# kevroy314/respmon

Measured on AMD Instinct MI355X. Metric: Eulerian-calibration frames/sec on 1080p x 256 buffer; achieved HBM GB/s, higher is better.
Workload: dtype f64

## Files before the change

### include/respmon_hip_debug.h

```cpp
#ifndef RESPMON_HIP_DEBUG_H
#define RESPMON_HIP_DEBUG_H

#include "respmon_hip.h"

#ifdef __cplusplus
extern "C" {
#endif

#define RM_FLAG_TINY_STORE 4u
#define RM_FLAG_TINY_STRIPS 8u
#define RM_FLAG_FF_PER_LEVEL 512u

int rm_debug_set(rm_ctx *ctx, const char *key, long long value);

int rm_debug_counters(rm_ctx *ctx, long long *out_host, void *stream);

const char *rm_debug_kernel_source_stamp(void);

int rm_debug_workspace(rm_ctx *ctx, const char *name, void *out_host, size_t bytes, void *stream);

int rm_debug_window_rows(rm_ctx *ctx, const rm_window *win, int row0, int nrows, double *out_host, void *stream);

#define RM_HOST_MARKS 5
int rm_debug_host_timeline(rm_ctx *ctx, double *out_host);

#define RM_ROI_PATH_NONE 0
#define RM_ROI_PATH_ONE_BLOB 1
#define RM_ROI_PATH_SCAN 2
#define RM_ROI_PATH_LABELLED 3
#define RM_ROI_PATH_AREA_BOUND 4
int rm_debug_roi_path(rm_ctx *ctx, int *path_out);

#ifdef __cplusplus
}
#endif
#endif
```

### respmon_amd/_capi.py

```python
import ctypes
import os

RM_OK = 0
RM_NO_CONTOUR = 1
RM_SPARSE_FALLBACK = 2
RM_COMM_ID_BYTES = 128
RM_EXCHANGE_SPARSE, RM_EXCHANGE_DENSE = 1, 2
RM_E_BADARG = -1
RM_E_UNSUPPORTED = -4
RM_E_COMM = -6
RM_E_BUSY = -7
RM_LOCATE_TICKETS = 2
RM_MAX_ROIS = 64
RM_U8, RM_F16, RM_F32, RM_F64 = 0, 1, 2, 3
RM_BGR8 = 4
RM_FLAG_NO_PRUNE = 1
RM_FLAG_UNFUSED_DOWN = 2
RM_FLAG_TINY_STORE = 4
RM_FLAG_TINY_STRIPS = 8
RM_FLAG_UNFUSED_SMALL = 16
RM_FLAG_CONTOUR_CLIP_FRAME = 32
RM_FLAG_FILTER_LAPLACIANS = 64
RM_FLAG_DENSE_SUM = 128
RM_FLAG_SPARSE_SUM = 256
RM_FLAG_FF_PER_LEVEL = 512

_c = ctypes
_vp, _i, _d, _sz, _u = _c.c_void_p, _c.c_int, _c.c_double, _c.c_size_t, _c.c_uint

SIGNATURES = {
    "rm_ctx_create": (_i, [_i, _c.POINTER(_vp)]),
    "rm_ctx_destroy": (_i, [_vp]),
    "rm_last_error_string": (_c.c_char_p, []),
    "rm_abi_version": (_i, []),
    "rm_ctx_workspace_bytes": (_sz, [_vp]),
    "rm_debug_set": (_i, [_vp, _c.c_char_p, _c.c_longlong]),
    "rm_profile_enable": (_i, [_vp, _i]),
    "rm_set_contour_clip_frame": (_i, [_vp, _i]),
    "rm_set_contour_labelling": (_i, [_vp, _i]),
    "rm_get_contour_clip_frame": (_i, [_vp, _c.POINTER(_i)]),
    "rm_get_contour_labelling": (_i, [_vp, _c.POINTER(_i)]),
    "rm_contour_stats": (_i, [_vp, _vp, _vp]),
    "rm_profile_read": (_i, [_vp, _vp, _c.POINTER(_i)]),
    "rm_debug_counters": (_i, [_vp, _vp, _vp]),
    "rm_debug_workspace": (_i, [_vp, _c.c_char_p, _vp, _c.c_size_t, _vp]),
    "rm_debug_kernel_source_stamp": (_c.c_char_p, []),
    "rm_debug_host_timeline": (_i, [_vp, _vp]),
    "rm_debug_roi_path": (_i, [_vp, _vp]),
    "rm_uint8_to_float": (_i, [_vp, _vp, _vp, _sz, _vp]),
    "rm_float_to_uint8": (_i, [_vp, _vp, _vp, _sz, _vp]),
    "rm_pyr_down": (_i, [_vp, _vp, _i, _i, _i, _i, _vp, _vp]),
    "rm_pyr_up": (_i, [_vp, _vp, _i, _i, _i, _vp, _i, _i, _i, _vp, _vp]),
    "rm_create_laplacian_video_pyramid": (_i, [_vp, _vp, _i, _i, _i, _i, _i, _c.POINTER(_vp), _vp]),
    "rm_collapse_laplacian_video_pyramid": (_i, [_vp, _c.POINTER(_vp), _i, _i, _i, _i, _vp, _vp]),
    "rm_temporal_bandpass_filter_fft": (_i, [_vp, _vp, _i, _sz, _d, _d, _d, _d, _vp, _vp]),
    "rm_temporal_operator": (_i, [_i, _d, _d, _d, _vp, _c.POINTER(_i), _c.POINTER(_i)]),
    "rm_time_average": (_i, [_vp, _vp, _i, _i, _sz, _vp, _vp]),
    "rm_lfilter": (_i, [_vp, _vp, _i, _sz, _vp, _vp, _i, _d, _vp, _vp]),
    "rm_threshold_mask": (_i, [_vp, _vp, _sz, _d, _vp, _vp, _vp]),
    "rm_eulerian_magnification_bandpass": (_i, [_vp, _vp, _i, _i, _i, _i, _d, _d, _d, _d, _i, _i, _d, _vp, _vp, _vp, _vp]),
    "rm_magnify": (_i, [_vp, _vp, _i, _i, _i, _i, _d, _d, _d, _d, _i, _i, _vp, _i, _vp]),
    "rm_magnify_bgr": (_i, [_vp, _vp, _i, _i, _i, _d, _d, _d, _d, _i, _i, _vp, _vp]),
    "rm_calibrate": (_i, [_vp, _vp, _i, _i, _i, _i, _d, _d, _d, _d, _i, _i, _d, _u, _vp, _vp, _vp]),
    "rm_heatmap_to_roi": (_i, [_vp, _vp, _i, _i, _i, _vp, _vp, _vp, _vp]),
    "rm_heat_sparse_packet_doubles": (_sz, [_i]),
    "rm_heat_sparse_pack": (_i, [_vp, _vp, _i, _i, _i, _vp, _vp]),
    "rm_heat_sparse_merge_roi": (_i, [_vp, _vp, _i, _i, _i, _i, _i, _i, _vp, _vp, _vp]),
    "rm_heat_sparse_tiles_needed": (_i, [_vp, _vp]),
    "rm_locate": (_i, [_vp, _vp, _i, _i, _i, _i, _d, _d, _d, _d, _i, _i, _d, _i, _u, _vp, _vp]),
    "rm_heatmap_to_rois": (_i, [_vp, _vp, _i, _i, _i, _i, _d, _vp, _vp, _c.POINTER(_i), _vp]),
    "rm_locate_multi": (_i, [_vp, _vp, _i, _i, _i, _i, _d, _d, _d, _d, _i, _i, _d, _i, _u, _i, _d, _vp, _vp, _c.POINTER(_i), _vp]),
    "rm_locate_submit": (_i, [_vp, _vp, _i, _i, _i, _i, _d, _d, _d, _d, _i, _i, _d, _i, _u, _vp, _vp]),
    "rm_locate_result": (_i, [_vp, _i, _vp]),
    "rm_shard_layout": (_i, [_i, _i, _i, _i, _c.POINTER(_sz)]),
    "rm_shard_layout_flags": (_i, [_i, _i, _i, _i, _c.c_uint, _c.POINTER(_sz)]),
    "rm_shard_pyramid": (_i, [_vp, _vp, _i, _i, _i, _i, _i, _i, _u, _vp, _vp]),
    "rm_shard_collapse": (_i, [_vp, _vp, _i, _i, _i, _i, _i, _d, _d, _d, _d, _i, _i, _d, _u, _vp, _vp]),
    "rm_shard_heat": (_i, [_vp, _vp, _d, _vp, _vp]),
    "rm_shard_finish": (_i, [_vp, _vp, _i, _i, _i, _i, _vp, _vp, _vp]),
    "rm_window_create": (_i, [_vp, _i, _i, _i, _i, _i, _u, _c.POINTER(_vp)]),
    "rm_window_destroy": (_i, [_vp]),
# ... 71 lines not shown
```

### respmon_amd/csrc/rm_ctx.hip

```cpp
#include "rm_internal.h"

using namespace rm;

static thread_local std::string g_err;

int fail(int code, const char *fmt, ...)
{
    char buf[512];
    va_list ap;
    va_start(ap, fmt);
    vsnprintf(buf, sizeof buf, fmt, ap);
    va_end(ap);
    g_err = buf;
    return code;
}

int ws_get(rm_ctx *ctx, const std::string &name, size_t bytes, void **out)
{
    DevBuf &b = ctx->bufs[name];
    if (b.cap < bytes) {
        if (b.p) {
            for (LocateTicket &t : ctx->tickets)
                if (t.active && t.done) HIP_TRY(hipEventSynchronize(t.done));
            const char *c = (const char *)ctx->dbg_cS, *p0 = (const char *)b.p;
            if (c && c >= p0 && c < p0 + b.cap) ctx->dbg_cS = nullptr;
            HIP_TRY(hipFree(b.p));
        }
        b.p = nullptr; b.cap = 0;
        size_t cap = (bytes + 255) / 256 * 256;
        HIP_TRY(hipMalloc(&b.p, cap));
        b.cap = cap;
    }
    *out = b.p;
    return RM_OK;
}

int ctx_stream_ok(rm_ctx *ctx, void *stream, const char *who)
{
    for (const LocateTicket &t : ctx->tickets)
        if (t.active && t.stream != (hipStream_t)stream)
            return fail(RM_E_BUSY, "%s: a rm_locate_submit of this context is in flight on another stream (fetch it with rm_locate_result first, or "
                                   "use its stream)", who);
    return RM_OK;
}

extern "C" int rm_debug_roi_path(rm_ctx *ctx, int *path_out)
{
    if (!ctx || !path_out) return fail(RM_E_BADARG, "rm_debug_roi_path: bad argument");
    *path_out = ctx->roi_path;
    return RM_OK;
}

extern "C" int rm_debug_host_timeline(rm_ctx *ctx, double *out)
{
    if (!ctx || !out) return fail(RM_E_BADARG, "rm_debug_host_timeline: bad argument");
    for (int i = 0; i < RM_HOST_MARKS; ++i) out[i] = ctx->host_marks[i];
    return RM_OK;
}

extern "C" int rm_abi_version(void) { return 1; }
extern "C" const char *rm_last_error_string(void) { return g_err.c_str(); }

extern "C" int rm_ctx_create(int device, rm_ctx **out)
{
    if (!out) return fail(RM_E_BADARG, "rm_ctx_create: out is NULL");
    HIP_TRY(hipSetDevice(device));
    rm_ctx *c = new rm_ctx();
    c->device = device;
    HIP_TRY(hipMalloc((void **)&c->d_state, sizeof(CollapseState)));
    HIP_TRY(hipHostMalloc((void **)&c->h_state, sizeof(CollapseState), hipHostMallocDefault));
    *out = c;
    return RM_OK;
}

extern "C" int rm_ctx_destroy(rm_ctx *ctx)
{
    if (!ctx) return RM_OK;
    (void)hipSetDevice(ctx->device);
    for (LocateTicket &t : ctx->tickets) {
        if (t.active && t.done) (void)hipEventSynchronize(t.done);
        if (t.done) (void)hipEventDestroy(t.done);
    }
// ... 21 lines not shown
    DebugKnobs &d = ctx->dbg;
    const std::string k(key);
    if (k == "temporal_valu") d.temporal_valu = (int)value;
    else if (k == "temporal_wide") d.temporal_wide = (int)value;
    else if (k == "dc_lds_front_end") d.dc_lds_front_end = (int)value;
    else if (k == "bgr_unfused") d.bgr_unfused = (int)value;
    else if (k == "no_fused_bounds") d.no_fused_bounds = (int)value;
    else if (k == "bounds_table_bytes") d.bounds_table_bytes = value;
    else if (k == "bounds_scalar") d.bounds_scalar = (int)value;
    else if (k == "bounds_l1") d.bounds_l1 = (int)value;
    else if (k == "bounds_up1") d.bounds_up1 = (int)value;
    else if (k == "dense_wf_list") d.dense_wf_list = (int)value;
    else if (k == "bounds_l1_rows") d.bounds_l1_rows = (int)value;
    else if (k == "dense_rows") d.dense_rows = (int)value;
    else if (k == "dense_general") d.dense_general = (int)value;
    else if (k == "dense_wave") d.dense_wave = (int)value;
    else if (k == "dense_frames") d.dense_frames = (int)value;
    else if (k == "dense_split") d.dense_split = (int)value;
    else if (k == "dc_segs") d.dc_segs = (int)value;
    else if (k == "dc_wpg") d.dc_wpg = (int)value;
    else if (k == "dc_split") d.dc_split = (int)value;
    else if (k == "dc_prio") d.dc_prio = (int)value;
    else if (k == "dc_prio_shift") d.dc_prio_shift = (int)value;
    else if (k == "store_slots") d.store_slots = value;
    else if (k == "store_default_slots") d.store_default_slots = value;
    else if (k == "collapse_fused") d.collapse_fused = (int)value;
    else if (k == "eval_fast") d.eval_fast = (int)value;
    else if (k == "exchange_dense") d.exchange_dense = (int)value;
    else if (k == "host_simple_shape") d.host_simple_shape = (int)value;
    else if (k == "host_area_bound") d.host_area_bound = (int)value;
    else if (k == "label_lazy") d.label_lazy = (int)value;
    else if (k == "heat_rows") d.heat_rows = (int)value;
    else if (k == "ff_parts") d.ff_parts = (int)value;
    else if (k == "heat_const_tiles") d.heat_const_tiles = (int)value;
    else if (k == "dense_t_low") d.dense_t_low = (int)value;
    else if (k == "dense_exact_top") d.dense_exact_top = (int)value;
    else if (k == "ccl_table") d.ccl_table = (int)value;
    else if (k == "ccl_tiles") d.ccl_tiles = (int)value;
    else if (k == "ccl_tile_waves") d.ccl_tile_waves = (int)value;
    else if (k == "label_host_steps") d.label_host_steps = value;
    else if (k == "flow_clip_bytes") d.flow_clip_bytes = value;
    else return fail(RM_E_BADARG, "rm_debug_set: unknown key '%s'", key);
    return RM_OK;
}

extern "C" int rm_profile_enable(rm_ctx *ctx, int on)
{
    if (!ctx) return fail(RM_E_BADARG, "rm_profile_enable: ctx is NULL");
    ctx->prof_mode = on < 0 ? 0 : on > 2 ? 2 : on;
    ctx->prof_on = on != 0;
    return RM_OK;
}

extern "C" int rm_profile_read(rm_ctx *ctx, double *ms, int *n)
{
    if (!ctx || !ms) return fail(RM_E_BADARG, "rm_profile_read: bad argument");
    for (int p = 0; p < RM_PROFILE_PHASES; ++p) {
        double total = ctx->prof_host_ms[p];
        ctx->prof_host_ms[p] = 0;
        std::vector<hipEvent_t> &v = ctx->prof_ev[p];
        if (p == 0) ctx->prof_sampled = (int)(v.size() / 2);
        for (size_t i = 0; i + 1 < v.size(); i += 2) {
            HIP_TRY(hipEventSynchronize(v[i + 1]));
            float t = 0.f;
            HIP_TRY(hipEventElapsedTime(&t, v[i], v[i + 1]));
            total += t;
// ... 132 lines not shown
```

### respmon_amd/csrc/rm_front.hip

```cpp
#include "rm_internal.h"

using namespace rm;


void pyr_geom(int H, int W, int levels, int skip, unsigned flags, PyrGeom &pg)
{
    level_sizes(H, W, levels, pg.h, pg.w);
    const int L = levels, S = skip;
    pg.L = L; pg.S = S;
    pg.all_zero = skip >= L - 1;
    if (pg.all_zero) { pg.S = 0; return; }
    pg.chain = S >= 1 && S <= 5 && !(flags & RM_FLAG_UNFUSED_DOWN);
    pg.off.assign(L, 0);
    pg.NP = 0;
    for (int l = S; l <= L - 2; ++l) { pg.off[l] = pg.NP; pg.NP += (size_t)pg.h[l] * pg.w[l]; }
    pg.lds_levels = 0;
    for (int l = S; l < L; ++l) pg.lds_levels += (size_t)pg.h[l] * pg.w[l];
    const size_t LDS_LIMIT = 150 * 1024;
    pg.fuse_small = pg.chain && !(flags & RM_FLAG_UNFUSED_SMALL) && L <= SMALL_MAX_LEVELS &&
                    pg.lds_levels * sizeof(double) <= LDS_LIMIT && pg.NP * sizeof(double) <= LDS_LIMIT;
    if (pg.fuse_small) {
        SmallGeom &sg = pg.sg;
        sg.S = S; sg.L = L; sg.NP = (int)pg.NP;
        int o = 0;
// ... 45 lines not shown
        g[S] = dst; cur = dst; cur_dtype = RM_F64;
        first = S + 1;
    }
    if (!pg.fuse_small) {
        for (int l = first; l < L; ++l) {
            double *dst = nullptr;
            if (l < S) RM_TRY(ws(ctx, (l & 1) ? "g_ping" : "g_pong", (size_t)T * h[l] * w[l], &dst));
            else RM_TRY(ws(ctx, "g" + std::to_string(l), (size_t)T * h[l] * w[l], &dst));
            {
                PhaseTimer pt(ctx, (l == 1) ? 0 : 1, s);
                RM_TRY(launch_pyr_down(cur, cur_dtype, T, h[l - 1], w[l - 1], dst, s));
            }
            g[l] = dst; cur = dst; cur_dtype = RM_F64;
        }
    }
    if (S == 0) {
        double *g0 = nullptr;
        RM_TRY(ws(ctx, "g0", (size_t)T * H * W, &g0));
        RM_TRY(launch_to_f64(frames, dtype, (size_t)T * H * W, g0, s));
        g[0] = g0;
    }
    PhaseTimer pt_small(ctx, 1, s);
    if (pg.fuse_small) {
        const size_t shmem = pg.lds_levels * sizeof(double);
        if (shmem > 64 * 1024)
            HIP_TRY(hipFuncSetAttribute((const void *)k_small_pyramid<>, hipFuncAttributeMaxDynamicSharedMemorySize, (int)shmem));
        hipLaunchKernelGGL(k_small_pyramid<>, dim3(T), dim3(SMALL_NT), shmem, s, (const double *)g[S], pg.sg, lap, ctx->d_state);
        LAUNCH_CHECK();
        ctx->state_fresh = true;
    } else {
        for (int l = L - 2; l >= S; --l)
            RM_TRY(launch_pyr_up(g[l + 1], T, h[l + 1], w[l + 1], lap + pg.off[l], h[l], w[l], 1, g[l], s, 0, NP, 0));
    }
    return RM_OK;
}

int front_filter(rm_ctx *ctx, const double *lap, int T, const PyrGeom &pg, double fps, double fmin, double fmax, double amp,
                        SmallLevels &out, hipStream_t s, int head)
{
    const std::vector<int> &h = pg.h, &w = pg.w;
    const int L = pg.L, S = pg.S;
    const size_t NP = pg.NP;
    const int Th = sym_frames(T);
    out.h = pg.h; out.w = pg.w; out.S = S; out.all_zero = false;
    const bool state_fresh = ctx->state_fresh;
    ctx->state_fresh = false;
    TemporalOp op;
    RM_TRY(get_operator(ctx, T, fps, fmin, fmax, &op, s));
    PhaseTimer pt_small(ctx, 1, s);
    double *bp = nullptr;
    RM_TRY(ws(ctx, "bp_all", (size_t)Th * NP, &bp));
    if (pg.filter_first) {
        RM_TRY(launch_temporal(ctx, lap, T, NP, op, amp, bp, s, ctx->d_state, false, head));
        ChainGeom cg;
        SmallLevels probe; probe.h = pg.h; probe.w = pg.w; probe.S = S;
        RM_TRY(make_geom(probe, cg));
        const long long npairs = (long long)cg.tiles_x * cg.tiles_y * Th;
        if (npairs >= (1ll << 31)) return fail(RM_E_UNSUPPORTED, "calibration: %lld (tile, frame) pairs exceed 2^31", npairs);
        double *dst = nullptr, *lo = nullptr, *hi = nullptr;
        int *sel_cnt = nullptr;
        RM_TRY(ws(ctx, "cS", (size_t)Th * NP, &dst));
        RM_TRY(ws(ctx, "tile_lo", (size_t)npairs, &lo));
        RM_TRY(ws(ctx, "tile_hi", (size_t)npairs, &hi));
        RM_TRY(ws(ctx, "sel_cnt", (size_t)cg.tiles_x * cg.tiles_y, &sel_cnt));
        const size_t sh = sizeof(double) * (pg.lds_levels + 2 * (size_t)h[S] * cg.tiles_x);
        if (sh > 64 * 1024)
            HIP_TRY(hipFuncSetAttribute((const void *)k_small_filter_first<>, hipFuncAttributeMaxDynamicSharedMemorySize, (int)sh));
        int cus_ff = 256;
#ifndef RM_HIPEMU
        HIP_TRY(hipDeviceGetAttribute(&cus_ff, hipDeviceAttributeMultiprocessorCount, ctx->device));
#endif
        int parts = (2 * Th <= cus_ff && cg.tiles_y >= 8) ? 2 : 1;
        if (ctx->dbg.ff_parts > 0) parts = std::min(ctx->dbg.ff_parts, std::max(1, cg.tiles_y / 2));
        hipLaunchKernelGGL(k_small_filter_first<>, dim3(Th * parts), dim3(SMALL_NT), sh, s, (const double *)bp, pg.sg, (int)pg.lds_levels, dst, ctx->d_state, cg,
                           cg.tiles_x * cg.tiles_y, lo, hi, sel_cnt, parts);
        LAUNCH_CHECK();
        out.state_ready = true; out.bounds_ready = true;
        out.cS = dst;
        return RM_OK;
    }
    if (pg.ff_levels) {
        RM_TRY(launch_temporal(ctx, lap, T, NP, op, amp, bp, s, ctx->d_state, false, head));
        out.state_ready = true;
        std::vector<double *> x(L, nullptr);
        x[S] = bp;
        const int depth = L - 1 - S;
        const bool fused_down = depth >= 1 && depth <= 5;
        auto level_buf = [&](int l) { return x[l] ? RM_OK : ws(ctx, "g" + std::to_string(l), (size_t)Th * h[l] * w[l], &x[l]); };
        RM_TRY(level_buf(L - 1));
        if (fused_down) {
            std::vector<int> hh(h.begin() + S, h.end()), ww(w.begin() + S, w.end());
            RM_TRY(launch_down_chain(ctx, bp, RM_F64, Th, hh, ww, depth, x[L - 1], s, false));
        } else {
            for (int l = S + 1; l < L; ++l) { RM_TRY(level_buf(l)); RM_TRY(launch_pyr_down(x[l - 1], RM_F64, Th, h[l - 1], w[l - 1], x[l], s)); }
        }
        double *dst = nullptr;
        RM_TRY(ws(ctx, "cS", (size_t)Th * NP, &dst));
        SmallLevels up; up.S = depth;
        up.h.assign(h.begin() + S, h.end()); up.w.assign(w.begin() + S, w.end());
        ChainGeom ug;
        if (depth >= 1 && depth < MAX_CHAIN && make_geom(up, ug) == RM_OK && (long long)ug.tiles_x * ug.tiles_y * Th < (1ll << 31)) {
            const int utiles = ug.tiles_x * ug.tiles_y, nitems = utiles * Th;
            const size_t sh = sizeof(double) * (size_t)ug.lds_total;
            if (sh > 64 * 1024) HIP_TRY(hipFuncSetAttribute((const void *)k_ff_collapse<>, hipFuncAttributeMaxDynamicSharedMemorySize, (int)sh));
            hipLaunchKernelGGL(k_ff_collapse<>, dim3((unsigned)std::min(nitems, 256 * 64)), dim3(64), sh, s, (const double *)bp, (const double *)x[L - 1],
                               ug, utiles, nitems, dst);
            LAUNCH_CHECK();
        } else {
// ... 118 lines not shown
```

### respmon_amd/csrc/rm_internal.h

```cpp
#pragma once
#include "../../include/respmon_hip.h"
#include "../../include/respmon_hip_debug.h"

#include <hip/hip_runtime.h>

#include <algorithm>
#include <atomic>
#include <chrono>
#include <cmath>
#include <cstdarg>
#include <cstdio>
#include <cstring>
#include <map>
#include <string>
#include <type_traits>
#include <vector>

#include "rm_contour.h"
#include "rm_kernels.h"
#include "rm_down_chain.h"
#include "rm_down_chain_u8.h"
#include "rm_dense_sum.h"
#include "rm_tile_eval.h"
#include "rm_bounds_l1.h"
// ... 36 lines not shown
    SumPlan sp{0, 0, 0, 0};
    bool l1_bounds = false;
};


struct DebugKnobs {
    int temporal_valu = 0;
    int temporal_wide = -1;
    int bgr_unfused = 0;
    int dc_lds_front_end = 0;
    int no_fused_bounds = 0;
    long long bounds_table_bytes = 0;
    int bounds_l1 = 2;
    int bounds_l1_rows = 0;
    int dense_wf_list = 1;
    int bounds_up1 = -1;
    int bounds_scalar = 0;
    int dense_rows = 0;
    int dense_general = 0;
    int dense_frames = 0;
    int dense_split = 0;
    int dense_wave = 1;
    int dc_segs = 0, dc_wpg = 0;
    int dc_prio_shift = 0;
    int dc_prio = 2;
    int dc_split = 0;
    int collapse_fused = 0;
    long long label_host_steps = 0;
    int ccl_tiles = 1;
    int ccl_tile_waves = 0;
    int ccl_table = -1;
    int heat_const_tiles = 1;
    int ff_parts = 0;
    int heat_rows = 1;
    int label_lazy = 1;
    int host_area_bound = 1;
    int host_simple_shape = 1;
    int exchange_dense = 0;
    int eval_fast = 1;
    int dense_exact_top = 1;
    int dense_t_low = -1;
    long long store_default_slots = 0;
    long long store_slots = 0;
    long long flow_clip_bytes = 0;
};

struct RoiSlot {
    uint8_t *h_bin = nullptr; size_t h_bin_cap = 0;
    uint8_t *h_rows_dirty = nullptr;
    CclComp *h_comps = nullptr; size_t h_comps_cap = 0;
    size_t dirty_w0 = 1, dirty_w1 = 0, dirty_geom = 0; int dirty_r0 = 0, dirty_r1 = -1;
    int *h_unserved = nullptr;
};
constexpr int ROI_SLOTS = 3;
struct RoiPending {
    int H = 0, W = 0, slot = 0; size_t nwords = 0, comps_cap = 0, rec_off = 0; bool label = false, clip = false, rows = false;
    bool lazy = false; hipStream_t stream = nullptr; const void *d_bits = nullptr, *d_list = nullptr;
};
struct LocateTicket {
    bool active = false;
    RoiPending roi;
    hipEvent_t done = nullptr;
    hipStream_t stream = nullptr;
    const void *frames = nullptr;
    int dtype = 0, T = 0, H = 0, W = 0, levels = 0, skip = 0, threshold = 0;
    double fps = 0, fmin = 0, fmax = 0, amp = 0, temporal_thr = 0;
    unsigned flags = 0;
    bool plan_valid = false;
};

struct rm_ctx {
    int device = 0;
    DebugKnobs dbg;
    std::map<std::string, DevBuf> bufs;
    CollapseState *d_state = nullptr;
    CollapseState *h_state = nullptr;
    RoiSlot slots[ROI_SLOTS];
    int cur_slot = 0;
    LocateTicket tickets[ROI_SLOTS - 1];
    bool tiles_const_once = false;
    bool clip_frame = false, clip_frame_once = false;
    int label_mode = -1, label_H = 0, label_W = 0, label_last_n = 0, label_used = 0;
    bool label_lazy = false;
    int roi_path = 0;
    long long label_unl_steps = -1;
    int label_unl_n = 0, label_streak = 0;
    int op_T = 0, op_nk = 0; double op_fps = 0, op_fmin = 0, op_fmax = 0;
    bool state_fresh = false;
    int op_mfma = 0;
    FlowWorkspace flow;
    CollapsePlan shard_plan;
    size_t eval_shmem = ~(size_t)0; int eval_per_cu = 0, eval_cus = 0;
    int nkept_H = 0, nkept_W = 0;
    int *h_flag = nullptr;
    void *comm = nullptr; int comm_rank = 0, comm_world = 1;
    ExchangeState xp_streams, xp_sharded;
    int refine_hint = 0;
    int dense_hint = 0;
    long long store_hint_slots = 0;
    const double *dbg_cS = nullptr; size_t dbg_cS_bytes = 0;
    long long dbg_pairs = 0, dbg_cap = 0, dbg_mine = 0; int dbg_mode = 0, dbg_auto_dense = 0, dbg_fused = 0;
    int prof_mode = 0;
    bool prof_on = false;
    int prof_calls = 0, prof_sampled = 0;
    std::vector<hipEvent_t> prof_ev[RM_PROFILE_PHASES];
    std::vector<hipEvent_t> prof_pool;
    double prof_host_ms[RM_PROFILE_PHASES] = {0, 0, 0, 0};
    double host_marks[RM_HOST_MARKS] = {0, 0, 0, 0, 0};
    std::chrono::steady_clock::time_point host_enter{}, host_last_return{};
    bool host_have_return = false;
};

static inline void host_mark(rm_ctx *c, int i)
{
    c->host_marks[i] = std::chrono::duration<double, std::micro>(std::chrono::steady_clock::now() - c->host_enter).count();
}

int ctx_stream_ok(rm_ctx *ctx, void *stream, const char *who);

struct PhaseTimer {
    rm_ctx *c; int phase; hipStream_t s; bool on;
    static hipEvent_t get(rm_ctx *c)
    {
        hipEvent_t e = nullptr;
        if (!c->prof_pool.empty()) { e = c->prof_pool.back(); c->prof_pool.pop_back(); }
// ... 33 lines not shown
    return (unsigned)(b > cap ? cap : b);
}
static inline bool valid_dtype(int d) { return d == RM_U8 || d == RM_F16 || d == RM_F32 || d == RM_F64; }
template <typename F> static inline void dispatch_dtype(int dtype, F &&f)
{
    switch (dtype) {
    case RM_U8: f(uint8_t()); break;
    case RM_F16: f(__half()); break;
    case RM_F32: f(float()); break;
    default: f(double()); break;
    }
}
static inline bool valid_buffer_dtype(int d) { return valid_dtype(d) || d == RM_BGR8; }
static inline int dtype_vec(int dtype) { return dtype == RM_F64 ? 2 : dtype == RM_F32 ? 4 : dtype == RM_F16 ? 8 : 16; }
static inline size_t dtype_size(int dtype) { return dtype == RM_F64 ? 8 : dtype == RM_F32 ? 4 : dtype == RM_F16 ? 2 : dtype == RM_BGR8 ? 3 : 1; }

int launch_bgr_to_gray(const uint8_t *bgr, size_t npix, uint8_t *gray, hipStream_t s);
int bgr_buffer_to_gray(rm_ctx *ctx, const void *frames, size_t npix, const void **gray_out, hipStream_t s);

int launch_pyr_down(const void *src, int dtype, int T, int h, int w, double *dst, hipStream_t s);
int launch_pyr_up(const double *src, int T, int sh, int sw, double *dst, int dh, int dw, int mode, const double *other, hipStream_t s,
                  size_t src_fs = 0, size_t dst_fs = 0, size_t other_fs = 0);
int launch_to_f64(const void *src, int dtype, size_t n, double *dst, hipStream_t s);
void level_sizes(int H, int W, int levels, std::vector<int> &h, std::vector<int> &w);

struct TemporalOp { const double *R = nullptr, *C = nullptr, *Rf = nullptr, *Cf = nullptr; int nk = 0, tiles = 0; };
int get_operator(rm_ctx *ctx, int T, double fps, double fmin, double fmax, TemporalOp *op, hipStream_t s);
int launch_temporal(rm_ctx *ctx, const double *x, int T, size_t NP, const TemporalOp &op, double amp, double *out, hipStream_t s,
                    rm::CollapseState *st_init = nullptr, bool full = false, int head = 0);

int launch_down_chain(rm_ctx *ctx, const void *frames, int dtype, int T, const std::vector<int> &h, const std::vector<int> &w, int S,
                      double *out, hipStream_t s, bool tiny);

struct SmallLevels {
    std::vector<int> h, w;
    int S = 0;
    const double *cS = nullptr;
    bool all_zero = false;
    bool state_ready = false;
    bool bounds_ready = false;
};

struct PyrGeom {
    std::vector<int> h, w;
    std::vector<size_t> off;
    size_t NP = 0;
    size_t lds_levels = 0;
    int S = 0, L = 0;
    bool all_zero = false;
    bool chain = false;
    bool fuse_small = false;
    bool filter_first = false;
    bool ff_levels = false;
    SmallGeom sg;
};

void pyr_geom(int H, int W, int levels, int skip, unsigned flags, PyrGeom &pg);
int front_pyramid(rm_ctx *ctx, const void *frames, int dtype, int T, int H, int W, const PyrGeom &pg, unsigned flags, double *lap, hipStream_t s);
int front_filter(rm_ctx *ctx, const double *lap, int T, const PyrGeom &pg, double fps, double fmin, double fmax, double amp, SmallLevels &out,
                 hipStream_t s, int head = 0);
int front_half(rm_ctx *ctx, const void *frames, int dtype, int T, int H, int W, double fps, double fmin, double fmax, double amp, int levels,
               int skip, unsigned flags, SmallLevels &out, hipStream_t s);
int make_geom(const SmallLevels &sl, rm::ChainGeom &g);

int launch_eval_pairs(rm_ctx *ctx, const CollapsePlan &cp, hipStream_t s);
int collapse_eval(rm_ctx *ctx, const SmallLevels &sl, int T, int t0, int t1, double thr, unsigned flags, CollapsePlan &cp, hipStream_t s);
// ... 14 lines not shown
```

### respmon_amd/csrc/rm_kernels.h

```cpp
#pragma once
#include <hip/hip_runtime.h>
#include <hip/hip_fp16.h>
#include <stdint.h>

#include <chrono>

#define RM_KERNEL template <int RM_UNIT_ = 0> __global__
#ifdef RM_HIPEMU
#define RM_VEC(T, N) T __attribute__((vector_size(sizeof(T) * (N))))
#else
#define RM_VEC(T, N) T __attribute__((ext_vector_type(N)))
#endif

namespace rm {

inline hipError_t stream_wait(hipStream_t s)
{
    const auto t0 = std::chrono::steady_clock::now();
    for (;;) {
        const hipError_t e = hipStreamQuery(s);
        if (e != hipErrorNotReady) return e;
        if (std::chrono::steady_clock::now() - t0 > std::chrono::milliseconds(4)) return hipStreamSynchronize(s);
    }
}
// ... 1093 lines not shown
            }
        }
    }
    double sm_mn = inf, sm_mx = -inf;
    if (have && lane < ntx && hS >= 3 && wS >= 3) {
        const int cand[2] = {p_mn, p_mx};
#pragma unroll
        for (int k = 0; k < 2; ++k) {
            if (cand[k] < 0) continue;
            int y = cand[k] / wS, x = cand[k] - y * wS;
            y = min(max(y, 1), hS - 2); x = min(max(x, 1), wS - 2);
            const double *r1 = p + (size_t)y * wS;
            const double v = lattice_sample(r1 - wS, r1, r1 + wS, x, g.lat_a, g.lat_b);
            sm_mn = (v < sm_mn) ? v : sm_mn; sm_mx = (v > sm_mx) ? v : sm_mx;
        }
    }
    lo_mn = wave_min(lo_mn); lo_mx = wave_max(lo_mx); hi_mn = wave_min(hi_mn); hi_mx = wave_max(hi_mx);
    sm_mn = wave_min(sm_mn); sm_mx = wave_max(sm_mx);
    if (lane == 0 && have) {
        const unsigned long long k_lo_mx = f64_key(lo_mx), k_lo_mn = f64_key(lo_mn), k_hi_mx = f64_key(hi_mx), k_hi_mn = f64_key(hi_mn);
        const int sp = (blockIdx.x + (blockIdx.y * 4 + wave) * 7) & (NSTRIPE - 1);
        striped_min_max(st->lb_min_keys, st->lb_max_keys, sp, k_lo_mn, k_lo_mx);
        striped_min_max(st->ub_min_keys, st->ub_max_keys, sp, k_hi_mn, k_hi_mx);
        if (sm_mn <= sm_mx) {
            const unsigned long long k_mn = f64_key(sm_mn), k_mx = f64_key(sm_mx);
            striped_min_max(st->smp_min_keys, st->smp_max_keys, sp, k_mn, k_mx);
        }
    }
}

__device__ __forceinline__ void frame_bounds_from_lds(const double *c, double *rmin_base, const SmallGeom &sg, const ChainGeom &g, int ntiles, int t,
                                                      double *cS, double *lo, double *hi, CollapseState *st, double (*s_red)[SMALL_NT / 64],
                                                      int (*s_arg)[SMALL_NT / 64], int mark_kid, int ty_a = 0, int ty_b = 0x7fffffff,
                                                      int y_lo = 0, int y_hi = 0x7fffffff, int y_out_a = 0, int y_out_b = 0x7fffffff)
{
    const int tid = threadIdx.x;
    const int S = sg.S;
    const int hS = sg.h[S], wS = sg.w[S], ntx = g.tiles_x;
    if (ty_b > g.tiles_y) ty_b = g.tiles_y;
    if (y_hi > hS - 1) y_hi = hS - 1;
    if (y_out_b > hS) y_out_b = hS;
    double *o = cS + (size_t)t * (hS * wS);
    const double inf = __builtin_huge_val();
    double c_mn = inf, c_mx = -inf;
    int i_mn = y_out_a * wS, i_mx = y_out_a * wS;
    for (int i = y_out_a * wS + tid; i < y_out_b * wS; i += SMALL_NT) {
        const double v = c[i];
        o[i] = v;
        if (v < c_mn) { c_mn = v; i_mn = i; }
        if (v > c_mx) { c_mx = v; i_mx = i; }
    }
    RM_TRACE_MARK(mark_kid, 8);
    double *rmin = rmin_base, *rmax = rmin + (size_t)hS * ntx;
    const float inv_ntx = 1.0f / (float)ntx;
    for (int i = y_lo * ntx + tid; i < (y_hi + 1) * ntx; i += SMALL_NT) {
        int y, tx;
        split_rc(i, ntx, inv_ntx, y, tx);
        const Region R = tile_region(g, tx, S);
        const double *row = c + y * wS;
        double mn = row[R.x0], mx = mn;
        for (int x = R.x0 + 1; x <= R.x1; ++x) {
            const double v = row[x];
            mn = (v < mn) ? v : mn;
            mx = (v > mx) ? v : mx;
        }
        rmin[i] = mn; rmax[i] = mx;
    }
    __syncthreads();
    RM_TRACE_MARK(mark_kid, 9);
    
    double lo_mn = inf, lo_mx = -inf, hi_mn = inf, hi_mx = -inf;
    (void)ntiles;
    for (int tile = ty_a * ntx + tid; tile < ty_b * ntx; tile += SMALL_NT) {
        const int tx = tile % ntx;
        const Region R = tile_region(g, tile, S);
        double mn = rmin[R.y0 * ntx + tx], mx = rmax[R.y0 * ntx + tx];
        for (int y = R.y0 + 1; y <= R.y1; ++y) {
            const double a = rmin[y * ntx + tx], b = rmax[y * ntx + tx];
            mn = (a < mn) ? a : mn;
            mx = (b > mx) ? b : mx;
        }
        lo[(size_t)t * ntiles + tile] = mn; hi[(size_t)t * ntiles + tile] = mx;
        lo_mn = (mn < lo_mn) ? mn : lo_mn; lo_mx = (mn > lo_mx) ? mn : lo_mx;
        hi_mn = (mx < hi_mn) ? mx : hi_mn; hi_mx = (mx > hi_mx) ? mx : hi_mx;
    }
    lo_mn = wave_min(lo_mn); lo_mx = wave_max(lo_mx); hi_mn = wave_min(hi_mn); hi_mx = wave_max(hi_mx);
    wave_arg_reduce(c_mn, i_mn, [](double o, double w) { return o < w; });
    wave_arg_reduce(c_mx, i_mx, [](double o, double w) { return o > w; });
    const int wave = tid >> 6;
    if ((tid & 63) == 0) {
        s_red[0][wave] = lo_mn; s_red[1][wave] = lo_mx; s_red[2][wave] = hi_mn; s_red[3][wave] = hi_mx;
        s_red[4][wave] = c_mn; s_red[5][wave] = c_mx; s_arg[0][wave] = i_mn; s_arg[1][wave] = i_mx;
    }
    __syncthreads();
    RM_TRACE_MARK(mark_kid, 11);
    if (wave != 0) return;
    {
        const bool have = tid < SMALL_NT / 64;
        lo_mn = have ? s_red[0][tid] : inf; lo_mx = have ? s_red[1][tid] : -inf;
        hi_mn = have ? s_red[2][tid] : inf; hi_mx = have ? s_red[3][tid] : -inf;
        c_mn = have ? s_red[4][tid] : inf; c_mx = have ? s_red[5][tid] : -inf;
        i_mn = have ? s_arg[0][tid] : 0; i_mx = have ? s_arg[1][tid] : 0;
        lo_mn = wave_min(lo_mn); lo_mx = wave_max(lo_mx); hi_mn = wave_min(hi_mn); hi_mx = wave_max(hi_mx);
        wave_arg_reduce(c_mn, i_mn, [](double o, double w) { return o < w; });
        wave_arg_reduce(c_mx, i_mx, [](double o, double w) { return o > w; });
    }
    if (tid == 0) {
        const unsigned long long k_lo_mx = f64_key(lo_mx), k_lo_mn = f64_key(lo_mn), k_hi_mx = f64_key(hi_mx), k_hi_mn = f64_key(hi_mn);
        const int sp = blockIdx.x & (NSTRIPE - 1);
        atomicMax(&st->lb_max_keys[sp], k_lo_mx);
        atomicMin(&st->lb_min_keys[sp], k_lo_mn);
// ... 8 lines not shown
            const double va = lattice_sample(ra - wS, ra, ra + wS, xa, g.lat_a, g.lat_b);
            const double vb = lattice_sample(rb - wS, rb, rb + wS, xb, g.lat_a, g.lat_b);
            atomicMin(&st->smp_min_keys[sp], f64_key(va < vb ? va : vb));
            atomicMax(&st->smp_max_keys[sp], f64_key(va > vb ? va : vb));
        }
    }
    RM_TRACE_MARK(mark_kid, 12);
}

RM_KERNEL __launch_bounds__(SMALL_NT) void k_small_collapse_bounds(const double *bp_all, SmallGeom sg, double *cS, CollapseState *st,
                                                                     ChainGeom g, int ntiles, double *lo, double *hi, int *sel_cnt)
{
    RM_TRACE_SCOPE(3);
    if (blockIdx.x == 0) for (int i = threadIdx.x; i < ntiles; i += SMALL_NT) sel_cnt[i] = 0;
    HIP_DYNAMIC_SHARED(double, lds)
    __shared__ double s_red[6][SMALL_NT / 64];
    __shared__ int s_arg[2][SMALL_NT / 64];
    const int t = blockIdx.x, tid = threadIdx.x;
    const int S = sg.S, L = sg.L;
    RM_TRACE_MARK(3, 0);
    fill_lds(lds, bp_all + (size_t)t * sg.NP, sg.NP, tid);
    __syncthreads();
    RM_TRACE_MARK(3, 1);
    for (int l = L - 3; l >= S; --l) {
        const int dh = sg.h[l], dw = sg.w[l], sh = sg.h[l + 1], sw = sg.w[l + 1];
        double *d = lds + sg.np_off[l];
        small_up_level(lds + sg.np_off[l + 1], sh, sw, dh, dw, tid, [&](int i, double v) { d[i] = v + d[i]; });
        __syncthreads();
        RM_TRACE_MARK(3, 2 + (L - 3 - l));
    }
    frame_bounds_from_lds(lds + sg.np_off[S], lds + sg.NP, sg, g, ntiles, t, cS, lo, hi, st, s_red, s_arg, 3);
}

RM_KERNEL __launch_bounds__(SMALL_NT) void k_small_filter_first(const double *xg, SmallGeom sg, int lds_levels, double *cS, CollapseState *st,
                                                                  ChainGeom g, int ntiles, double *lo, double *hi, int *sel_cnt, int parts)
{
    RM_TRACE_SCOPE(3);
    if (blockIdx.x == 0) for (int i = threadIdx.x; i < ntiles; i += SMALL_NT) sel_cnt[i] = 0;
    HIP_DYNAMIC_SHARED(double, lds)
    __shared__ double s_red[6][SMALL_NT / 64];
    __shared__ int s_arg[2][SMALL_NT / 64];
    const int t = blockIdx.x / parts, part = blockIdx.x - t * parts, tid = threadIdx.x;
    const int S = sg.S, L = sg.L;
    const int nS = sg.h[S] * sg.w[S];
    const int ty_a = (int)((long long)g.tiles_y * part / parts), ty_b = (int)((long long)g.tiles_y * (part + 1) / parts);
    const int y_lo = parts == 1 ? 0 : tile_region(g, ty_a * g.tiles_x, S).y0;
    const int y_hi = parts == 1 ? sg.h[S] - 1 : tile_region(g, (ty_b - 1) * g.tiles_x, S).y1;
    const int y_out_a = part == 0 ? 0 : min(sg.h[S], (ty_a * CT_H) >> S), y_out_b = part == parts - 1 ? sg.h[S] : min(sg.h[S], (ty_b * CT_H) >> S);
    RM_TRACE_MARK(3, 0);
    fill_lds(lds + sg.g_off[S], xg + (size_t)t * nS, nS, tid);
    __syncthreads();
    RM_TRACE_MARK(3, 1);
    for (int l = S + 1; l < L; ++l) {
        const int sh = sg.h[l - 1], sw = sg.w[l - 1], dh = sg.h[l], dw = sg.w[l];
        const double *sp = lds + sg.g_off[l - 1];
        double *d = lds + sg.g_off[l];
        for (int x = (tid & 63); x < dw; x += 64) {
            const int c0 = reflect101(2 * x - 2, sw), c1 = reflect101(2 * x - 1, sw), c2 = reflect101(2 * x, sw);
            const int c3 = reflect101(2 * x + 1, sw), c4 = reflect101(2 * x + 2, sw);
            for (int y = (tid >> 6); y < dh; y += SMALL_NT / 64) {
                double r[5];
#pragma unroll
                for (int k = 0; k < 5; ++k) {
                    const double *row = sp + reflect101(2 * y - 2 + k, sh) * sw;
                    r[k] = row[c2] * 6 + (row[c1] + row[c3]) * 4 + row[c0] + row[c4];
                }
                d[y * dw + x] = (r[2] * 6 + (r[1] + r[3]) * 4 + r[0] + r[4]) * (1.0 / 256);
            }
        }
        __syncthreads();
    }
    RM_TRACE_MARK(3, 2);
    for (int l = L - 2; l >= S; --l) {
        const int dh = sg.h[l], dw = sg.w[l], sh = sg.h[l + 1], sw = sg.w[l + 1];
        double *d = lds + sg.g_off[l];
        const bool last = l == S;
        small_up_level(lds + sg.g_off[l + 1], sh, sw, dh, dw, tid, [&](int i, double v) { d[i] = last ? d[i] - v : v; }, last ? y_lo : 0,
                       last ? y_hi + 1 : 0x7fffffff);
        __syncthreads();
    }
    RM_TRACE_MARK(3, 4);
    frame_bounds_from_lds(lds + sg.g_off[S], lds + lds_levels, sg, g, ntiles, t, cS, lo, hi, st, s_red, s_arg, 3, ty_a, ty_b, y_lo, y_hi, y_out_a, y_out_b);
}

constexpr double PRUNE_REL_MARGIN = 1e-12;

constexpr int SLOT_PRUNED = -1;
constexpr unsigned long long DENSE_ONE_IN = 2;
struct SumPlan {
    int mode;
    unsigned int cap_slots;
    unsigned int npairs_mine;
    int auto_dense_ok;
};
__device__ __forceinline__ bool sum_is_dense(const CollapseState *st, const SumPlan &sp)
{
    const unsigned int kept = st->n_slots;
    if (sp.mode == 1 || kept > sp.cap_slots) return true;
    if (sp.mode == 2) return false;
    return sp.auto_dense_ok && (unsigned long long)kept * DENSE_ONE_IN > (unsigned long long)sp.npairs_mine;
}

__device__ __forceinline__ unsigned long long block_excl_scan_256(unsigned long long v, unsigned long long *s_wave, unsigned long long &total)
{
    const int lane = threadIdx.x & 63, wave = threadIdx.x >> 6;
    unsigned long long inc = v;
#pragma unroll
    for (int d = 1; d < 64; d <<= 1) {
        const unsigned long long o = __shfl_up(inc, d);
        if (lane >= d) inc += o;
    }
    if (lane == 63) s_wave[wave] = inc;
    __syncthreads();
    unsigned long long base = 0, tot = 0;
#pragma unroll
// ... 940 lines not shown
```

Measured before the change: 320,300.

## Compact small-pyramid LDS layout into dead rows to raise filter-first occupancy

Adds a compact LDS layout for the filter-first kernel. The coarser pyramid levels and the per-row min/max tables are placed in rows of the base level that fall outside this block's part, and the first downsampled level is carried in registers across a barrier. This shrinks dynamic shared memory per block so more blocks can be resident, and the host chooses the part count and layout from an occupancy query. The cost is extra offset arithmetic, an added barrier, and more complex legality checks. By default (-1) the compact layout is used only when it increases blocks per CU, but FF_MAX_PER_CU=1 caps that gain, so it may rarely activate.

```diff
diff --git a/include/respmon_hip_debug.h b/include/respmon_hip_debug.h
--- a/include/respmon_hip_debug.h
+++ b/include/respmon_hip_debug.h
@@ -31,6 +31,8 @@
 #define RM_ROI_PATH_AREA_BOUND 4
 int rm_debug_roi_path(rm_ctx *ctx, int *path_out);
 
+int rm_debug_small_pyramid_plan(rm_ctx *ctx, int out[4]);
+
 #ifdef __cplusplus
 }
 #endif
diff --git a/respmon_amd/_capi.py b/respmon_amd/_capi.py
--- a/respmon_amd/_capi.py
+++ b/respmon_amd/_capi.py
@@ -47,6 +47,7 @@
     "rm_debug_kernel_source_stamp": (_c.c_char_p, []),
     "rm_debug_host_timeline": (_i, [_vp, _vp]),
     "rm_debug_roi_path": (_i, [_vp, _vp]),
+    "rm_debug_small_pyramid_plan": (_i, [_vp, _vp]),
     "rm_uint8_to_float": (_i, [_vp, _vp, _vp, _sz, _vp]),
     "rm_float_to_uint8": (_i, [_vp, _vp, _vp, _sz, _vp]),
     "rm_pyr_down": (_i, [_vp, _vp, _i, _i, _i, _i, _vp, _vp]),
diff --git a/respmon_amd/csrc/rm_ctx.hip b/respmon_amd/csrc/rm_ctx.hip
--- a/respmon_amd/csrc/rm_ctx.hip
+++ b/respmon_amd/csrc/rm_ctx.hip
@@ -48,6 +48,13 @@
 {
     if (!ctx || !path_out) return fail(RM_E_BADARG, "rm_debug_roi_path: bad argument");
     *path_out = ctx->roi_path;
+    return RM_OK;
+}
+
+extern "C" int rm_debug_small_pyramid_plan(rm_ctx *ctx, int *out)
+{
+    if (!ctx || !out) return fail(RM_E_BADARG, "rm_debug_small_pyramid_plan: bad argument");
+    for (int i = 0; i < 4; ++i) out[i] = ctx->ff_plan[i];
     return RM_OK;
 }
 
@@ -135,6 +142,7 @@
     else if (k == "label_lazy") d.label_lazy = (int)value;
     else if (k == "heat_rows") d.heat_rows = (int)value;
     else if (k == "ff_parts") d.ff_parts = (int)value;
+    else if (k == "ff_compact") d.ff_compact = (int)value;
     else if (k == "heat_const_tiles") d.heat_const_tiles = (int)value;
     else if (k == "dense_t_low") d.dense_t_low = (int)value;
     else if (k == "dense_exact_top") d.dense_exact_top = (int)value;
diff --git a/respmon_amd/csrc/rm_front.hip b/respmon_amd/csrc/rm_front.hip
--- a/respmon_amd/csrc/rm_front.hip
+++ b/respmon_amd/csrc/rm_front.hip
@@ -101,6 +101,23 @@
         for (int l = L - 2; l >= S; --l)
             RM_TRY(launch_pyr_up(g[l + 1], T, h[l + 1], w[l + 1], lap + pg.off[l], h[l], w[l], 1, g[l], s, 0, NP, 0));
     }
+    return RM_OK;
+}
+
+static int ff_resident(rm_ctx *ctx, size_t bytes, int *per_cu, int *cus)
+{
+    auto it = ctx->ff_occ.find(bytes);
+    if (it == ctx->ff_occ.end()) {
+        int n = 0, c = 256;
+#ifndef RM_HIPEMU
+        HIP_TRY(hipOccupancyMaxActiveBlocksPerMultiprocessor(&n, (const void *)k_small_filter_first<>, SMALL_NT, bytes));
+        HIP_TRY(hipDeviceGetAttribute(&c, hipDeviceAttributeMultiprocessorCount, ctx->device));
+#else
+        n = (int)std::min<size_t>(2, (160 * 1024) / (bytes + 1024));
+#endif
+        it = ctx->ff_occ.emplace(bytes, std::make_pair(std::max(1, n), std::max(1, c))).first;
+    }
+    *per_cu = it->second.first; *cus = it->second.second;
     return RM_OK;
 }
 
@@ -132,17 +149,33 @@
         RM_TRY(ws(ctx, "tile_lo", (size_t)npairs, &lo));
         RM_TRY(ws(ctx, "tile_hi", (size_t)npairs, &hi));
         RM_TRY(ws(ctx, "sel_cnt", (size_t)cg.tiles_x * cg.tiles_y, &sel_cnt));
-        const size_t sh = sizeof(double) * (pg.lds_levels + 2 * (size_t)h[S] * cg.tiles_x);
+        const size_t sh_old = sizeof(double) * (pg.lds_levels + 2 * (size_t)h[S] * cg.tiles_x), sh_compact = sizeof(double) * (size_t)h[S] * w[S];
+        const int max_parts = std::max(1, cg.tiles_y / 2);
+        int cus_ff = 256, per_cu = 1;
+        auto layout = [&](int p, bool &compact, size_t &bytes) -> int {
+            int old_cu = 1, new_cu = 1;
+            RM_TRY(ff_resident(ctx, sh_old, &old_cu, &cus_ff));
+            compact = ctx->dbg.ff_compact != 0 && ff_compact_legal(pg.sg, cg, p);
+            if (compact) RM_TRY(ff_resident(ctx, sh_compact, &new_cu, &cus_ff));
+            if (compact && ctx->dbg.ff_compact < 0 && std::min(new_cu, FF_MAX_PER_CU) <= old_cu) compact = false;
+            bytes = compact ? sh_compact : sh_old; per_cu = compact ? new_cu : old_cu;
+            return RM_OK;
+        };
+        int parts = 1;
+        bool compact = false;
+        size_t sh = sh_old;
+        if (ctx->dbg.ff_parts > 0) parts = std::min(ctx->dbg.ff_parts, max_parts);
+        else if (cg.tiles_y >= 8)
+            for (int p = std::min(FF_MAX_PARTS, max_parts); p >= 2 && parts == 1; --p) {
+                RM_TRY(layout(p, compact, sh));
+                if ((long long)p * Th <= (long long)std::min(per_cu, FF_MAX_PER_CU) * cus_ff) parts = p;
+            }
+        RM_TRY(layout(parts, compact, sh));
         if (sh > 64 * 1024)
             HIP_TRY(hipFuncSetAttribute((const void *)k_small_filter_first<>, hipFuncAttributeMaxDynamicSharedMemorySize, (int)sh));
-        int cus_ff = 256;
-#ifndef RM_HIPEMU
-        HIP_TRY(hipDeviceGetAttribute(&cus_ff, hipDeviceAttributeMultiprocessorCount, ctx->device));
-#endif
-        int parts = (2 * Th <= cus_ff && cg.tiles_y >= 8) ? 2 : 1;
-        if (ctx->dbg.ff_parts > 0) parts = std::min(ctx->dbg.ff_parts, std::max(1, cg.tiles_y / 2));
+        ctx->ff_plan[0] = parts; ctx->ff_plan[1] = compact ? 1 : 0; ctx->ff_plan[2] = (int)sh; ctx->ff_plan[3] = per_cu;
         hipLaunchKernelGGL(k_small_filter_first<>, dim3(Th * parts), dim3(SMALL_NT), sh, s, (const double *)bp, pg.sg, (int)pg.lds_levels, dst, ctx->d_state, cg,
-                           cg.tiles_x * cg.tiles_y, lo, hi, sel_cnt, parts);
+                           cg.tiles_x * cg.tiles_y, lo, hi, sel_cnt, parts, compact ? 1 : 0);
         LAUNCH_CHECK();
         out.state_ready = true; out.bounds_ready = true;
         out.cS = dst;
diff --git a/respmon_amd/csrc/rm_internal.h b/respmon_amd/csrc/rm_internal.h
--- a/respmon_amd/csrc/rm_internal.h
+++ b/respmon_amd/csrc/rm_internal.h
@@ -92,6 +92,7 @@
     int ccl_table = -1;
     int heat_const_tiles = 1;
     int ff_parts = 0;
+    int ff_compact = -1;
     int heat_rows = 1;
     int label_lazy = 1;
     int host_area_bound = 1;
@@ -151,6 +152,8 @@
     FlowWorkspace flow;
     CollapsePlan shard_plan;
     size_t eval_shmem = ~(size_t)0; int eval_per_cu = 0, eval_cus = 0;
+    std::map<size_t, std::pair<int, int>> ff_occ;
+    int ff_plan[4] = {0, 0, 0, 0};
     int nkept_H = 0, nkept_W = 0;
     int *h_flag = nullptr;
     void *comm = nullptr; int comm_rank = 0, comm_world = 1;
@@ -250,6 +253,8 @@
 int launch_down_chain(rm_ctx *ctx, const void *frames, int dtype, int T, const std::vector<int> &h, const std::vector<int> &w, int S,
                       double *out, hipStream_t s, bool tiny);
 
+constexpr int FF_MAX_PARTS = 2;
+constexpr int FF_MAX_PER_CU = 1;
 struct SmallLevels {
     std::vector<int> h, w;
     int S = 0;
diff --git a/respmon_amd/csrc/rm_kernels.h b/respmon_amd/csrc/rm_kernels.h
--- a/respmon_amd/csrc/rm_kernels.h
+++ b/respmon_amd/csrc/rm_kernels.h
@@ -1149,7 +1149,8 @@
 __device__ __forceinline__ void frame_bounds_from_lds(const double *c, double *rmin_base, const SmallGeom &sg, const ChainGeom &g, int ntiles, int t,
                                                       double *cS, double *lo, double *hi, CollapseState *st, double (*s_red)[SMALL_NT / 64],
                                                       int (*s_arg)[SMALL_NT / 64], int mark_kid, int ty_a = 0, int ty_b = 0x7fffffff,
-                                                      int y_lo = 0, int y_hi = 0x7fffffff, int y_out_a = 0, int y_out_b = 0x7fffffff)
+                                                      int y_lo = 0, int y_hi = 0x7fffffff, int y_out_a = 0, int y_out_b = 0x7fffffff,
+                                                      double *rmax_base = nullptr, int tbl_row0 = 0)
 {
     const int tid = threadIdx.x;
     const int S = sg.S;
@@ -1168,7 +1169,8 @@
         if (v > c_mx) { c_mx = v; i_mx = i; }
     }
     RM_TRACE_MARK(mark_kid, 8);
-    double *rmin = rmin_base, *rmax = rmin + (size_t)hS * ntx;
+    double *rmin = rmin_base, *rmax = rmax_base ? rmax_base : rmin + (size_t)hS * ntx;
+    const int tb = tbl_row0 * ntx;
     const float inv_ntx = 1.0f / (float)ntx;
     for (int i = y_lo * ntx + tid; i < (y_hi + 1) * ntx; i += SMALL_NT) {
         int y, tx;
@@ -1181,7 +1183,7 @@
             mn = (v < mn) ? v : mn;
             mx = (v > mx) ? v : mx;
         }
-        rmin[i] = mn; rmax[i] = mx;
+        rmin[i - tb] = mn; rmax[i - tb] = mx;
     }
     __syncthreads();
     RM_TRACE_MARK(mark_kid, 9);
@@ -1191,9 +1193,9 @@
     for (int tile = ty_a * ntx + tid; tile < ty_b * ntx; tile += SMALL_NT) {
         const int tx = tile % ntx;
         const Region R = tile_region(g, tile, S);
-        double mn = rmin[R.y0 * ntx + tx], mx = rmax[R.y0 * ntx + tx];
+        double mn = rmin[R.y0 * ntx + tx - tb], mx = rmax[R.y0 * ntx + tx - tb];
         for (int y = R.y0 + 1; y <= R.y1; ++y) {
-            const double a = rmin[y * ntx + tx], b = rmax[y * ntx + tx];
+            const double a = rmin[y * ntx + tx - tb], b = rmax[y * ntx + tx - tb];
             mn = (a < mn) ? a : mn;
             mx = (b > mx) ? b : mx;
         }
@@ -1268,8 +1270,72 @@
     frame_bounds_from_lds(lds + sg.np_off[S], lds + sg.NP, sg, g, ntiles, t, cS, lo, hi, st, s_red, s_arg, 3);
 }
 
+constexpr int FF_CARRY = 4;
+
+__host__ __device__ inline void ff_part_rows(const SmallGeom &sg, const ChainGeom &g, int part, int parts, int &ty_a, int &ty_b, int &y_lo, int &y_hi)
+{
+    const int S = sg.S;
+    ty_a = (int)((long long)g.tiles_y * part / parts); ty_b = (int)((long long)g.tiles_y * (part + 1) / parts);
+    y_lo = parts == 1 ? 0 : tile_region(g, ty_a * g.tiles_x, S).y0;
+    y_hi = parts == 1 ? sg.h[S] - 1 : tile_region(g, (ty_b - 1) * g.tiles_x, S).y1;
+}
+
+__host__ __device__ __forceinline__ int ff_dead_fit(int n, int &a, int a_end, int &b, int b_end)
+{
+    int off = -1;
+    if (a + n <= a_end) { off = a; a += n; }
+    else if (b + n <= b_end) { off = b; b += n; }
+    return off;
+}
+
+__host__ __device__ inline int ff_compact_level_off(const SmallGeom &sg, int y_lo, int y_hi, int l)
+{
+    const int S = sg.S, wS = sg.w[S];
+    int a = 0, b = (y_hi + 1) * wS, off = -1;
+    for (int k = S + 1; k <= l; ++k) {
+        off = ff_dead_fit(sg.h[k] * sg.w[k], a, y_lo * wS, b, sg.h[S] * wS);
+        if (off < 0) return -1;
+    }
+    return off;
+}
+
+__host__ __device__ inline bool ff_compact_table_off(const SmallGeom &sg, int y_lo, int y_hi, int ntx, int &rmin_off, int &rmax_off)
+{
+    const int S = sg.S, wS = sg.w[S], n = (y_hi - y_lo + 1) * ntx;
+    int a = 0, b = (y_hi + 1) * wS;
+    rmin_off = ff_dead_fit(n, a, y_lo * wS, b, sg.h[S] * wS);
+    rmax_off = ff_dead_fit(n, a, y_lo * wS, b, sg.h[S] * wS);
+    return rmin_off >= 0 && rmax_off >= 0;
+}
+
+__host__ __device__ inline bool ff_compact_legal(const SmallGeom &sg, const ChainGeom &g, int parts)
+{
+    const int S = sg.S;
+    if (parts < 2 || S + 1 >= sg.L || sg.g_off[S] != 0) return false;
+    if (sg.h[S + 1] * sg.w[S + 1] > FF_CARRY * SMALL_NT || sg.w[S + 1] > 1024) return false;
+    for (int part = 0; part < parts; ++part) {
+        int ty_a, ty_b, y_lo, y_hi, o_mn, o_mx;
+        ff_part_rows(sg, g, part, parts, ty_a, ty_b, y_lo, y_hi);
+        if (ff_compact_level_off(sg, y_lo, y_hi, sg.L - 1) < 0 || !ff_compact_table_off(sg, y_lo, y_hi, g.tiles_x, o_mn, o_mx)) return false;
+    }
+    return true;
+}
+
+__device__ __forceinline__ double small_down_at(const double *sp, int sh, int sw, int y, int x)
+{
+    const int c0 = reflect101(2 * x - 2, sw), c1 = reflect101(2 * x - 1, sw), c2 = reflect101(2 * x, sw);
+    const int c3 = reflect101(2 * x + 1, sw), c4 = reflect101(2 * x + 2, sw);
+    double r[5];
+#pragma unroll
+    for (int k = 0; k < 5; ++k) {
+        const double *row = sp + reflect101(2 * y - 2 + k, sh) * sw;
+        r[k] = row[c2] * 6 + (row[c1] + row[c3]) * 4 + row[c0] + row[c4];
+    }
+    return (r[2] * 6 + (r[1] + r[3]) * 4 + r[0] + r[4]) * (1.0 / 256);
+}
+
 RM_KERNEL __launch_bounds__(SMALL_NT) void k_small_filter_first(const double *xg, SmallGeom sg, int lds_levels, double *cS, CollapseState *st,
-                                                                  ChainGeom g, int ntiles, double *lo, double *hi, int *sel_cnt, int parts)
+                                                                  ChainGeom g, int ntiles, double *lo, double *hi, int *sel_cnt, int parts, int compact)
 {
     RM_TRACE_SCOPE(3);
     if (blockIdx.x == 0) for (int i = threadIdx.x; i < ntiles; i += SMALL_NT) sel_cnt[i] = 0;
@@ -1279,18 +1345,44 @@
     const int t = blockIdx.x / parts, part = blockIdx.x - t * parts, tid = threadIdx.x;
     const int S = sg.S, L = sg.L;
     const int nS = sg.h[S] * sg.w[S];
-    const int ty_a = (int)((long long)g.tiles_y * part / parts), ty_b = (int)((long long)g.tiles_y * (part + 1) / parts);
-    const int y_lo = parts == 1 ? 0 : tile_region(g, ty_a * g.tiles_x, S).y0;
-    const int y_hi = parts == 1 ? sg.h[S] - 1 : tile_region(g, (ty_b - 1) * g.tiles_x, S).y1;
+    int ty_a, ty_b, y_lo, y_hi;
+    ff_part_rows(sg, g, part, parts, ty_a, ty_b, y_lo, y_hi);
     const int y_out_a = part == 0 ? 0 : min(sg.h[S], (ty_a * CT_H) >> S), y_out_b = part == parts - 1 ? sg.h[S] : min(sg.h[S], (ty_b * CT_H) >> S);
+    auto level = [&](int l) { return lds + ((compact && l > S) ? ff_compact_level_off(sg, y_lo, y_hi, l) : sg.g_off[l]); };
     RM_TRACE_MARK(3, 0);
     fill_lds(lds + sg.g_off[S], xg + (size_t)t * nS, nS, tid);
     __syncthreads();
     RM_TRACE_MARK(3, 1);
-    for (int l = S + 1; l < L; ++l) {
+    int l_first = S + 1;
+    if (compact) {
+        const int sh = sg.h[S], sw = sg.w[S], dh = sg.h[S + 1], dw = sg.w[S + 1];
+        const double *sp = lds + sg.g_off[S];
+        const float inv_dw = 1.0f / (float)dw;
+        double keep[FF_CARRY];
+#pragma unroll
+        for (int k = 0; k < FF_CARRY; ++k) {
+            const int i = tid + k * SMALL_NT;
+            keep[k] = 0.0;
+            if (i < dh * dw) {
+                int y, x;
+                split_rc(i, dw, inv_dw, y, x);
+                keep[k] = small_down_at(sp, sh, sw, y, x);
+            }
+        }
+        __syncthreads();
+        double *d = level(S + 1);
+#pragma unroll
+        for (int k = 0; k < FF_CARRY; ++k) {
+            const int i = tid + k * SMALL_NT;
+            if (i < dh * dw) d[i] = keep[k];
+        }
+        __syncthreads();
+        l_first = S + 2;
+    }
+    for (int l = l_first; l < L; ++l) {
         const int sh = sg.h[l - 1], sw = sg.w[l - 1], dh = sg.h[l], dw = sg.w[l];
-        const double *sp = lds + sg.g_off[l - 1];
-        double *d = lds + sg.g_off[l];
+        const double *sp = level(l - 1);
+        double *d = level(l);
         for (int x = (tid & 63); x < dw; x += 64) {
             const int c0 = reflect101(2 * x - 2, sw), c1 = reflect101(2 * x - 1, sw), c2 = reflect101(2 * x, sw);
             const int c3 = reflect101(2 * x + 1, sw), c4 = reflect101(2 * x + 2, sw);
@@ -1309,14 +1401,17 @@
     RM_TRACE_MARK(3, 2);
     for (int l = L - 2; l >= S; --l) {
         const int dh = sg.h[l], dw = sg.w[l], sh = sg.h[l + 1], sw = sg.w[l + 1];
-        double *d = lds + sg.g_off[l];
+        double *d = level(l);
         const bool last = l == S;
-        small_up_level(lds + sg.g_off[l + 1], sh, sw, dh, dw, tid, [&](int i, double v) { d[i] = last ? d[i] - v : v; }, last ? y_lo : 0,
+        small_up_level(level(l + 1), sh, sw, dh, dw, tid, [&](int i, double v) { d[i] = last ? d[i] - v : v; }, last ? y_lo : 0,
                        last ? y_hi + 1 : 0x7fffffff);
         __syncthreads();
     }
     RM_TRACE_MARK(3, 4);
-    frame_bounds_from_lds(lds + sg.g_off[S], lds + lds_levels, sg, g, ntiles, t, cS, lo, hi, st, s_red, s_arg, 3, ty_a, ty_b, y_lo, y_hi, y_out_a, y_out_b);
+    int rmin_off = lds_levels, rmax_off = lds_levels + sg.h[S] * g.tiles_x, tbl_row0 = 0;
+    if (compact) { (void)ff_compact_table_off(sg, y_lo, y_hi, g.tiles_x, rmin_off, rmax_off); tbl_row0 = y_lo; }
+    frame_bounds_from_lds(lds + sg.g_off[S], lds + rmin_off, sg, g, ntiles, t, cS, lo, hi, st, s_red, s_arg, 3, ty_a, ty_b, y_lo, y_hi, y_out_a, y_out_b,
+                          lds + rmax_off, tbl_row0);
 }
 
 constexpr double PRUNE_REL_MARGIN = 1e-12;
```

Result: slower. 302,500 (-5.6%).
